# angelocatalani/neural-network-compression

Measured on AMD Instinct MI355X. Metric: weights/sec through prune+k-means (K=256), higher is better.
Workload: dtype f32

## Files before the change

neural_network_compression_amd/csrc/nnc_hip.hip:

```cpp
#include "nnc_common.hpp"
#include "nnc_km_shared.hpp"


extern "C" size_t nnc_kmeans_workspace_bytes(int32_t k)
{
    (void)k;
    return sizeof(KmWs) + 256;
}

extern "C" int32_t nnc_fix_shift(float absmax, int64_t n_total)
{
    int L = 1;
    while (((int64_t)1 << L) < n_total && L < 62) L++;
    if (!(absmax > 0.0f) || !std::isfinite(absmax)) return 0;
    int P = 0;
    (void)std::frexp((double)absmax, &P);
    return std::min(28, 62 - L) - P;
}

__device__ __forceinline__ int fix_f32(float v, int Sft)
{
    return (int)rintf(ldexpf(v, Sft));
}

// ... 911 lines not shown
        tab = &ws->tab[ws->cur];
        src.zr = ws->bnd.zr; src.zl = ws->bnd.zl; src.cand = ws->bnd.cand; src.orig = ws->bnd.orig; src.ku = &ws->bnd.ku;
    }
    KmBndPre<BR> pre;
    const bool fixed_src = !(which & 1);
    if (fixed_src) km_bounds_preload<BR>(pre, j, lane, ws, src);
    const int stop = (which & 2) ? 0 : (ws->st.done | ws->st.paused);
    const int unasked = (which & 4) ? !ws->wide : 0;
    const int hint = ws->help_hint;
    const float mean = ws->p.x_mean;
    const int Sft = ws->p.fix_shift;
    if (stop | unasked) return;
    int qn_seen = 0;
    if (!fixed_src) km_bounds_preload<BR>(pre, j, lane, ws, src);
    const bool published = km_bounds_wave<BR>(j, lane, xs, n, ws, tab, src, mean, Sft, pblk, &qn_seen, pre, hint == 2, &wg_searched);
    KBSTAMP(16 * j + 5, 0);
    const bool waits = hint == 2 && !published && fixed_src;
    int looks = 0;
    if (waits) {
        const int nwaves = pre.ku;
        for (int nap = 0; nap < 64 && __builtin_amdgcn_s_memrealtime() - t_enter < 900ull; nap++) __builtin_amdgcn_s_sleep(16);
        for (int look = 0; look < 128; look++) {
            looks++;
            if (km_peek_i(&ws->q_searched) >= nwaves) break;
            __builtin_amdgcn_s_sleep(48);
        }
    }
    KBSTAMP(16 * j + 7, 0);
    if (NNC_KM_TRACE_PTR && lane == 0) NNC_KM_TRACE_PTR[16 * j + 12] = (unsigned long long)looks;
    if (published || hint || uni_i(qn_seen) > 0) km_bounds_help(lane, xs, ws, tab, mean, Sft, j, hint == 2 ? pre.ku : 0);
    KBSTAMP(16 * j + 6, 0);
}

__global__ __launch_bounds__(256) void k_prefix_blocks(const float *__restrict__ xs, long long n, float mean, int Sft, long long *__restrict__ pblk)
{
    const int lane = threadIdx.x & 63;
    const long long nblk = (n + KM_PB - 1) / KM_PB;
    long long *__restrict__ pfine = pblk + km_pfine_off(n);
    const long long wave = (long long)blockIdx.x * 4 + (threadIdx.x >> 6), nwaves = (long long)gridDim.x * 4;
    for (long long b0 = wave; b0 < nblk; b0 += 4 * nwaves) {
        float4 v[4];
        bool full[4], have[4];
#pragma unroll
        for (int u = 0; u < 4; u++) {
            const long long b = b0 + u * nwaves;
            have[u] = b < nblk;
            full[u] = have[u] && (b + 1) * KM_PB <= n;
            v[u] = full[u] ? *reinterpret_cast<const float4 *>(xs + b * KM_PB + 4 * lane) : make_float4(0.f, 0.f, 0.f, 0.f);
        }
#pragma unroll
        for (int u = 0; u < 4; u++) {
            if (!have[u]) continue;
            const long long b = b0 + u * nwaves;
            const long long i0 = b * KM_PB + 4 * lane;
            long long acc = 0;
            if (full[u]) {
                acc = ((long long)fix_f32(v[u].x - mean, Sft) + fix_f32(v[u].y - mean, Sft)) + ((long long)fix_f32(v[u].z - mean, Sft) + fix_f32(v[u].w - mean, Sft));
            } else {
                for (int q = 0; q < 4; q++) if (i0 + q < n) acc += fix_f32(xs[i0 + q] - mean, Sft);
            }
#pragma unroll
            for (int off = 1; off <= 8; off <<= 1) acc += __shfl_xor(acc, off);
            if ((lane & 15) == 0) pfine[4 * b + (lane >> 4)] = acc;
            acc += __shfl_xor(acc, 16);
            acc += __shfl_xor(acc, 32);
            if (lane == 0) pblk[b] = acc;
        }
    }
    if (blockIdx.x == 0 && threadIdx.x == 0) pblk[nblk] = 0;
}

__global__ __launch_bounds__(256) void k_prefix_fine(long long *__restrict__ pblk, long long n)
{
    const long long nblk = km_prefix_nblk(n);
    const long long *__restrict__ pgrp = km_pgrp(pblk, n);
    long long *__restrict__ pfine = pblk + km_pfine_off(n);
    const long long b = (long long)blockIdx.x * 256 + threadIdx.x;
    if (b > nblk) return;
    const long long base = pblk[b] + pgrp[b / KM_PG];
    if (b == nblk) { pfine[4 * b] = base; return; }
    const long long q0 = pfine[4 * b], q1 = pfine[4 * b + 1], q2 = pfine[4 * b + 2];
    pfine[4 * b] = base; pfine[4 * b + 1] = base + q0; pfine[4 * b + 2] = base + q0 + q1; pfine[4 * b + 3] = base + q0 + q1 + q2;
}

__global__ __launch_bounds__(KM_THREADS) void k_prefix_groups(long long *__restrict__ pblk, long long nblk, long long *__restrict__ pgrp)
{
    __shared__ long long wave_tot[KM_THREADS / 64];
// ... 998 lines not shown
    HIPCHK(hipMemcpy(out8, reinterpret_cast<KmWs *>(ws)->kl_trace, 24 * sizeof(unsigned long long), hipMemcpyDeviceToHost));
    return NNC_OK;
}

extern "C" int nnc_debug_set_trace(unsigned long long *buf_dev)
{
    HIPCHK(hipMemcpyToSymbol(HIP_SYMBOL(g_km_trace), &buf_dev, sizeof(buf_dev)));
    unsigned long long *fin = buf_dev ? buf_dev + 6 * 1024 : nullptr;
    HIPCHK(hipMemcpyToSymbol(HIP_SYMBOL(g_fin_trace), &fin, sizeof(fin)));
    return NNC_OK;
}

extern "C" int nnc_debug_clock(int blocks, int iters, float *out_dev, void *stream)
{
    hipLaunchKernelGGL(k_debug_clock, dim3(blocks), dim3(256), 0, S(stream), iters, out_dev);
    LAUNCHCHK("k_debug_clock");
    return NNC_OK;
}

static int g_ablation = 0;
static int g_deal = []() { const char *e = getenv("NNC_KM_DEAL"); return e ? atoi(e) : 1; }();
extern "C" int nnc_debug_set_ablation(int a) { g_ablation = a; return NNC_OK; }
#else
static const int g_ablation = 0, g_deal = 1;
#endif

extern "C" size_t nnc_kmeans_prefix_bytes(int64_t n)
{
    if (n < 0) return 0;
    const long long nblk = (n + KM_PB - 1) / KM_PB;
    return (size_t)(nblk + 2 + (nblk + 1 + KM_PG - 1) / KM_PG + 2 + 4 * (nblk + 1) + 4) * sizeof(long long);
}

extern "C" int nnc_kmeans_prefix_build(const float *x_sorted, const nnc_kmeans_params *p, int64_t *prefix_dev, void *stream)
{
    if (!p || !prefix_dev || p->n < 0 || (p->n > 0 && !x_sorted)) return fail(NNC_EINVAL, "nnc_kmeans_prefix_build: bad argument");
    if ((reinterpret_cast<uintptr_t>(x_sorted) & 15) != 0 || (reinterpret_cast<uintptr_t>(prefix_dev) & 7) != 0)
        return fail(NNC_EINVAL, "nnc_kmeans_prefix_build: x_sorted must be 16-byte aligned, prefix_dev 8-byte aligned");
    if (p->n >= ((int64_t)1 << 40)) return fail(NNC_EINVAL, "nnc_kmeans_prefix_build: n >= 2^40");
    const long long nblk = (p->n + KM_PB - 1) / KM_PB;
    long long *pb = reinterpret_cast<long long *>(prefix_dev);
    const int grid = (int)std::max<long long>(1, std::min<long long>((nblk + 3) / 4, (long long)cu_count() * 8));
    NNC_LAUNCH_PROF(NNC_PROF_PREFIX, k_prefix_blocks, dim3(grid), dim3(256), 0, S(stream), x_sorted, (long long)p->n, p->x_mean, p->fix_shift, pb);
    LAUNCHCHK("k_prefix_blocks");
    const long long ngroups = (nblk + 1 + KM_PG - 1) / KM_PG;
    long long *pg = pb + nblk + 2;
    if (ngroups > 0) {
        hipLaunchKernelGGL(k_prefix_groups, dim3((unsigned)ngroups), dim3(KM_THREADS), 0, S(stream), pb, nblk, pg);
        LAUNCHCHK("k_prefix_groups");
    }
    hipLaunchKernelGGL(k_prefix_top, dim3(1), dim3(KM_THREADS), 0, S(stream), pg, ngroups);
    LAUNCHCHK("k_prefix_top");
    hipLaunchKernelGGL(k_prefix_fine, dim3((unsigned)((nblk + 1 + 255) / 256)), dim3(256), 0, S(stream), pb, (long long)p->n);
    LAUNCHCHK("k_prefix_fine");
    return NNC_OK;
}

int km_launch_accumulate(const float *x, KmWs *w, const nnc_kmeans_params *p, void *stream, int which)
{
    if (p->prefix_dev && p->n > 0) {
        if ((reinterpret_cast<uintptr_t>(x) & 15) != 0) return fail(NNC_EINVAL, "rank-boundary iteration: the sorted vector must be 16-byte aligned");
        const int nb = (p->k + 3) / 4;
        const long long *pb = reinterpret_cast<const long long *>(p->prefix_dev);
#define KM_LAUNCH_BOUNDS(BR) NNC_LAUNCH_PROF(NNC_PROF_BOUNDS, (k_bounds<BR>), dim3(nb), dim3(256), 0, S(stream), x, (long long)p->n, w, which, pb)
        if (p->k <= 64) KM_LAUNCH_BOUNDS(1);
        else if (p->k <= 128) KM_LAUNCH_BOUNDS(2);
        else if (p->k <= 256) KM_LAUNCH_BOUNDS(4);
        else if (p->k <= 512) KM_LAUNCH_BOUNDS(8);
        else if (p->k <= 1024) KM_LAUNCH_BOUNDS(16);
        else KM_LAUNCH_BOUNDS(KM_BND_R);
#undef KM_LAUNCH_BOUNDS
        LAUNCHCHK("k_bounds");
        return NNC_OK;
    }
    int glog2, rlog2;
    km_defaults(p, &glog2, &rlog2);
// ... 1386 lines not shown
```

neural_network_compression_amd/csrc/nnc_layer.hip:

```cpp
#include <hip/hip_runtime.h>

#include <algorithm>
#include <cmath>
#include <cstdint>
#include <cstring>
#include <string>
#include <vector>

#include "nnc.h"

int nnc_set_error_(int code, const char *msg);
int nnc_publish_bytes_(const void *src_dev, void *dst_host_mapped, int nbytes, void *host_ticket, uint64_t ticket, void *stream);
int nnc_wait_ticket_(void *host_ticket, uint64_t ticket, void *stream);
int nnc_sort_pruned_bounded_flagged_(const float *x, int64_t n, int64_t n_neg, int64_t n_zero, float vmin, float vmax, float thr,
                                     float *sorted_out, void *ws, size_t ws_bytes, int32_t *flag_dev, void *stream);

extern "C" int nnc_host_linspace_f32(float start, float stop, int32_t num, float *out)
{
    if (num < 0 || (num > 0 && !out)) return nnc_set_error_(NNC_EINVAL, "nnc_host_linspace_f32: bad argument");
    if (num == 0) return NNC_OK;
    const int div = num - 1;
    const volatile float delta = stop - start;
    if (div > 0) {
        const volatile float step = delta / (float)div;
        for (int i = 0; i < num; i++) {
            volatile float y = (float)i;
            if (step == 0.0f) { y = y / (float)div; y = y * delta; }
            else y = y * step;
            y = y + start;
            out[i] = y;
        }
        out[num - 1] = stop;
    } else {
        volatile float y = 0.0f;
        y = y * delta;
        y = y + start;
        out[0] = y;
    }
    return NNC_OK;
}

static void linspace_f64(double start, double stop, int num, double *out)
{
    const int div = num - 1;
    const volatile double delta = stop - start;
    if (div > 0) {
        const volatile double step = delta / (double)div;
        for (int i = 0; i < num; i++) {
// ... 243 lines not shown
            if (!std::isfinite(min_nz)) {
                LHIP(hipStreamWaitEvent(s, side->join, 0));
                LHIP(hipStreamSynchronize(s));
                side_join.joined = true;
                if (lp->prune) { res->sigma = h_prune[0]; res->threshold = h_prune[1]; res->n_zeroed = h_nz[0]; }
                res->status = NNC_LAYER_HOST;
                return NNC_OK;
            }
            LCHK(nnc_host_linspace_f32(min_nz, max_nz, 32, steps));
            std::memcpy(h_steps, steps, 128);
            LCHK(nnc_rank_sorted_f32(xs, n, h_steps, 32, ranks_d, stream));
        }
        const uint64_t t_rk = ++(*ticket_io);
        LCHK(nnc_publish_bytes_(out6 + 2, hb + 512 + 8, 56 + 33 * 8 + 16, h_ticket, t_rk, stream));
        LCHK(nnc_wait_ticket_(h_ticket_side, t_mv, side->stream));
        LHIP(hipStreamWaitEvent(s, side->join, 0));
        side_join.joined = true;
        const float mean = h_mv[0], var = h_mv[1];
        if (!std::isfinite(mean) || !std::isfinite(var) || !std::isfinite(xmin) || !std::isfinite(xmax)) {
            LCHK(nnc_wait_ticket_(h_ticket, t_rk, stream));
            if (lp->prune) { res->sigma = h_prune[0]; res->threshold = h_prune[1]; res->n_zeroed = h_nz[0]; }
            res->status = NNC_LAYER_HOST;
            return NNC_OK;
        }
        nnc_kmeans_params p;
        std::memset(&p, 0, sizeof(p));
        const volatile float tol = var * 1e-4f;
        const volatile float lo = xmin - mean, hi = xmax - mean;
        p.n = n; p.n_total = n; p.k = k; p.max_iter = 300;
        p.fix_shift = nnc_fix_shift(std::max(std::fabs((float)lo), std::fabs((float)hi)), n);
        p.grid_log2 = 0; p.replicas_log2 = -1; p.flags = lp->km_flags & (NNC_KM_TWO_LAUNCH | NNC_KM_LOOP);
        p.x_mean = mean; p.tol = tol; p.lo = lo; p.hi = hi;
        if (with_prefix) {
            LCHK(nnc_kmeans_prefix_build(xs, &p, reinterpret_cast<int64_t *>(wb + L.prefix), stream));
            p.prefix_dev = reinterpret_cast<int64_t *>(wb + L.prefix);
        }
        LCHK(nnc_wait_ticket_(h_ticket, t_rk, stream));
        if (bounded && *h_oob) {
            if (lp->prune) { res->sigma = h_prune[0]; res->threshold = h_prune[1]; res->n_zeroed = h_nz[0]; }
            res->status = NNC_LAYER_HOST;
            return NNC_OK;
        }
        if (lp->mode == NNC_INIT_LINEAR) {
            LCHK(nnc_host_linspace_f32(xmin, xmax, k, space));
        } else {
            int64_t counts31[31];
            for (int b = 0; b < 31; b++) counts31[b] = h_ranks[b + 1] - h_ranks[b];
            for (int b = 0; b < 31; b++)
                if (steps[b] <= 0.0f && 0.0f < steps[b + 1]) { counts31[b] -= n_zero; break; }
            float xnew[300];
            double cdf[300];
            LCHK(nnc_host_cdf(steps, counts31, xnew, cdf));
            LCHK(nnc_host_density_init(xnew, cdf, lp->bits, space));
        }
        std::memcpy(h_space, space, (size_t)k * 4);
        LCHK(nnc_kmeans_init(wb + L.km_ws, L.km_ws_bytes, &p, h_space, stream));
        nnc_kmeans_status st;
        std::memset(&st, 0, sizeof(st));
        int32_t nwin = 0;
        LCHK(nnc_kmeans_fit(xs, wb + L.km_ws, &p, 16, 1, L.reloc_bytes ? wb + L.reloc : nullptr, L.reloc_bytes, hb, ticket_io, &st, &nwin, stream));
        if (!st.done) {
            if (lp->prune) { res->sigma = h_prune[0]; res->threshold = h_prune[1]; res->n_zeroed = h_nz[0]; }
            res->status = NNC_LAYER_HOST;
            return NNC_OK;
        }
        LCHK(nnc_kmeans_get_centers(wb + L.km_ws, 0, 0, centers_d, stream));
        LCHK(nnc_kmeans_assign(x, wb + L.km_ws, &p, 0, labels_out, res->label_bytes, lp->want_values ? values_out : nullptr, nullptr, nullptr, stream));
// ... 15 lines not shown
```

neural_network_compression_amd/csrc/nnc_sort.hip:

```cpp
#include <hip/hip_runtime.h>
#include <cmath>
#include <cstdlib>
#include <cstring>

#include <algorithm>
#include <string>

#include "nnc.h"

extern "C" const char *nnc_last_error(void);
int nnc_set_error_(int code, const char *msg);

#ifndef OS_THREADS
#define OS_THREADS 1024
#endif
#define OS_WAVES (OS_THREADS / 64)
#ifndef OS_ITEMS
#define OS_ITEMS 16
#endif
#ifndef OS_BLOCKS_PER_CU
#define OS_BLOCKS_PER_CU 1
#endif
#ifndef OS_RANK_LDS
#define OS_RANK_LDS 1
#endif
#define OS_TILE (OS_THREADS * OS_ITEMS)
#define OS_MAXBITS 9
#define OS_MAXR (1 << OS_MAXBITS)
#define OS_MAXPASS 4
#define OS_SPIN_LIMIT (1 << 22)
#define OSP_THREADS 1024
#define OSP_PER 16
#define OSP_TILE (OSP_THREADS * OSP_PER)

__device__ __forceinline__ unsigned f32_ord(float v)
{
    const unsigned b = __float_as_uint(v);
    return (b & 0x80000000u) ? ~b : (b | 0x80000000u);
}
__device__ __forceinline__ float f32_unord(unsigned o)
{
    return __uint_as_float((o & 0x80000000u) ? (o ^ 0x80000000u) : ~o);
}

struct OsMap { unsigned lo_neg, hi_neg, lo_pos, hi_pos, span_neg; int bounded; };
struct OsPlan { int passes; int shift[OS_MAXPASS]; int rb[OS_MAXPASS]; };

__device__ __forceinline__ unsigned os_key(const OsMap &m, float e, bool &outside)
{
    const unsigned o = f32_ord(e);
    if (!m.bounded) return o;
    if (e < 0.0f) { outside |= (o < m.lo_neg) | (o > m.hi_neg); const unsigned c = o < m.lo_neg ? m.lo_neg : (o > m.hi_neg ? m.hi_neg : o); return c - m.lo_neg; }
    outside |= (o < m.lo_pos) | (o > m.hi_pos);
    const unsigned c = o < m.lo_pos ? m.lo_pos : (o > m.hi_pos ? m.hi_pos : o);
    return m.span_neg + (c - m.lo_pos);
}
__device__ __forceinline__ float os_value(const OsMap &m, unsigned k)
{
    if (!m.bounded) return f32_unord(k);
    return f32_unord(k < m.span_neg ? k + m.lo_neg : k - m.span_neg + m.lo_pos);
}

#define OS_CTRL_WORDS 4

template <bool SKIPZ>
__global__ __launch_bounds__(OSP_THREADS) void k_os_prep(const float *__restrict__ x, long long n, unsigned *__restrict__ keys,
                                                         unsigned long long *__restrict__ ctrl, long long cap, OsMap km, int rb0, unsigned *__restrict__ ghist)
{
    __shared__ unsigned comp_s[SKIPZ ? OSP_TILE : 1];
    __shared__ unsigned hist_s[OS_MAXR];
    __shared__ unsigned wave_tot[OSP_THREADS / 64];
    __shared__ unsigned long long base_s;
    const int tid = threadIdx.x, lane = tid & 63, wv = tid >> 6;
    for (int i = tid; i < OS_MAXR; i += OSP_THREADS) hist_s[i] = 0u;
    __syncthreads();
    const bool vec = (reinterpret_cast<uintptr_t>(x) & 15) == 0;
    const float4 *x4 = reinterpret_cast<const float4 *>(x);
    const unsigned mask0 = (1u << rb0) - 1u;
    bool outside = false;
    const long long ntiles = (n + OSP_TILE - 1) / OSP_TILE;
    auto load_tile = [&](long long tt, float (&e)[OSP_PER]) {
        const long long tile0 = tt * OSP_TILE;
        if (tt >= ntiles) return;
        if (vec && tile0 + OSP_TILE <= n) {
#pragma unroll
            for (int j = 0; j < OSP_PER / 4; j++) {
                const float4 q = x4[(tile0 >> 2) + (long long)j * OSP_THREADS + tid];
                e[4 * j] = q.x; e[4 * j + 1] = q.y; e[4 * j + 2] = q.z; e[4 * j + 3] = q.w;
            }
        } else {
#pragma unroll
            for (int j = 0; j < OSP_PER; j++) {
                const long long i = tile0 + (long long)j * OSP_THREADS + tid;
                e[j] = i < n ? x[i] : 0.0f;
            }
        }
    };
    float en[OSP_PER];
    load_tile(blockIdx.x, en);
    for (long long t = blockIdx.x; t < ntiles; t += gridDim.x) {
        const long long tile0 = t * OSP_TILE;
        const bool fast = vec && tile0 + OSP_TILE <= n;
        float e[OSP_PER];
#pragma unroll
        for (int j = 0; j < OSP_PER; j++) e[j] = en[j];
        load_tile(t + gridDim.x, en);
        unsigned key[OSP_PER];
        unsigned take = 0;
#pragma unroll
        for (int j = 0; j < OSP_PER; j++) {
            bool ok = SKIPZ ? !(e[j] == 0.0f) : true;
            if (!SKIPZ && !fast) ok = tile0 + (long long)j * OSP_THREADS + tid < n;
            key[j] = 0u;
            if (ok) { key[j] = os_key(km, e[j], outside); take |= 1u << j; }
        }
#pragma unroll
        for (int j = 0; j < OSP_PER; j++)
            if (take & (1u << j)) atomicAdd(&hist_s[key[j] & mask0], 1u);
        if (SKIPZ) {
            const unsigned c = (unsigned)__popc(take);
            unsigned sc = c;
            for (int off = 1; off < 64; off <<= 1) { const unsigned o = __shfl_up(sc, off); if (lane >= off) sc += o; }
            if (lane == 63) wave_tot[wv] = sc;
            __syncthreads();
            unsigned pre = 0, tot = 0;
            for (int w = 0; w < OSP_THREADS / 64; w++) { const unsigned o = wave_tot[w]; if (w < wv) pre += o; tot += o; }
            if (tid == 0) base_s = atomicAdd(ctrl, (unsigned long long)tot);
            unsigned at = pre + sc - c;
#pragma unroll
            for (int j = 0; j < OSP_PER; j++)
                if (take & (1u << j)) comp_s[at++] = key[j];
            __syncthreads();
            const long long base = (long long)base_s;
            for (unsigned i = tid; i < tot; i += OSP_THREADS)
                if (base + i < cap) keys[base + i] = comp_s[i];
            __syncthreads();
        }
    }
    if (outside) atomicOr(ctrl + 1, 1ull);
    __syncthreads();
    for (int i = tid; i < OS_MAXR; i += OSP_THREADS) {
        const unsigned v = hist_s[i];
        if (v) atomicAdd(&ghist[i], v);
    }
}

#ifdef NNC_DIAG
__device__ unsigned long long *g_os_trace = nullptr;
extern "C" int nnc_debug_os_trace(void *buf)
{
    unsigned long long *p = reinterpret_cast<unsigned long long *>(buf);
    return hipMemcpyToSymbol(HIP_SYMBOL(g_os_trace), &p, sizeof(p)) == hipSuccess ? NNC_OK : NNC_EHIP;
}
#define OS_STAMP(i) do { if (g_os_trace && t == 0) g_os_trace[((size_t)pass * 8192 + (size_t)(tile < 8192 ? tile : 8191)) * 8 + (i)] = __builtin_amdgcn_s_memrealtime(); } while (0)
#else
#define OS_STAMP(i) do { } while (0)
#endif

__device__ __forceinline__ void os_publish(unsigned long long *w, unsigned tag, unsigned v)
{
    __hip_atomic_store(w, ((unsigned long long)tag << 32) | v, __ATOMIC_RELAXED, __HIP_MEMORY_SCOPE_AGENT);
}
__device__ __forceinline__ unsigned long long os_peek(const unsigned long long *w)
{
    return __hip_atomic_load(w, __ATOMIC_RELAXED, __HIP_MEMORY_SCOPE_AGENT);
}

template <int RB, bool FULL>
__device__ __forceinline__ void os_peers(unsigned d, bool valid, unsigned &plo, unsigned &phi)
{
    const unsigned long long all = FULL ? ~0ull : __ballot(valid);
    plo = (unsigned)all; phi = (unsigned)(all >> 32);
#pragma unroll
    for (int b = 0; b < RB; b++) {
        const int m = ((int)(d << (31 - b))) >> 31;
        const unsigned long long mb = FULL ? __ballot(m != 0) : __ballot(valid && m != 0);
        plo &= ~((unsigned)mb ^ (unsigned)m);
        phi &= ~((unsigned)(mb >> 32) ^ (unsigned)m);
    }
}

#ifndef OS_LOOK
#define OS_LOOK 4
#endif

template <int RB, int SRC, int DST>
__global__ __launch_bounds__(OS_THREADS, OS_BLOCKS_PER_CU * OS_THREADS / 256) void k_os_pass(const void *__restrict__ in_, void *__restrict__ out_, long long n, int shift, int pass, int nrb,
                                                           const unsigned *__restrict__ ghist, unsigned *__restrict__ ghist_next, unsigned long long *__restrict__ status,
                                                           unsigned long long *__restrict__ ctrl, OsMap km, long long n_neg, long long n_zero, int abl)
{
    constexpr int R = 1 << RB;
    constexpr unsigned MASK = (unsigned)R - 1u;
    constexpr int DPT = (R + OS_THREADS - 1) / OS_THREADS;
    __shared__ unsigned keys_s[OS_TILE];
    __shared__ unsigned short wcnt[OS_WAVES][R];
    __shared__ unsigned short tpre[R];
    __shared__ unsigned gpos[R];
    __shared__ unsigned gdig[R];
    __shared__ unsigned nhist[OS_MAXR];
    __shared__ unsigned wsum[OS_WAVES];
    __shared__ long long tile_s;
    const int t = threadIdx.x, lane = t & 63, wv = t >> 6;
    const unsigned *in_k = reinterpret_cast<const unsigned *>(in_);
    const float *in_f = reinterpret_cast<const float *>(in_);
    unsigned *out_k = reinterpret_cast<unsigned *>(out_);
    float *out_f = reinterpret_cast<float *>(out_);
    const unsigned tagA = 2u * (unsigned)pass + 1u, tagP = tagA + 1u;
    unsigned *ticket = reinterpret_cast<unsigned *>(ctrl + 2) + pass;
    const int nshift = shift + RB;
    const unsigned nmask = nrb > 0 ? (1u << nrb) - 1u : 0u;
    {
        unsigned v[DPT], own = 0;
#pragma unroll
        for (int r = 0; r < DPT; r++) { const int d = t * DPT + r; v[r] = d < R ? ghist[d] : 0u; own += v[r]; }
        unsigned sc = own;
        for (int off = 1; off < 64; off <<= 1) { const unsigned o = __shfl_up(sc, off); if (lane >= off) sc += o; }
        if (lane == 63) wsum[wv] = sc;
        for (int i = t; i < OS_MAXR; i += OS_THREADS) nhist[i] = 0u;
        __syncthreads();
        unsigned run = sc - own;
        for (int w = 0; w < wv; w++) run += wsum[w];
#pragma unroll
        for (int r = 0; r < DPT; r++) { const int d = t * DPT + r; if (d < R) gdig[d] = run; run += v[r]; }
// ... 144 lines not shown
                            __builtin_amdgcn_s_sleep(1);
                        } else polls = 0;
                    }
                }
                os_publish(&status[(size_t)tile * R + d], tagP, excl + tc[r]);
            }
            gpos[d] = gdig[d] + excl - (unsigned)tpre[d];
        }
        OS_STAMP(4);
        __syncthreads();
        OS_STAMP(5);
        for (int j = t; j < cnt_tile; j += OS_THREADS) {
            const unsigned kv = keys_s[j];
            const unsigned d = (kv >> shift) & MASK;
            const unsigned r = gpos[d] + (unsigned)j;
            if ((long long)r < n && !(abl & 4)) {
                if (DST == 0) out_k[r] = kv;
                else out_f[(long long)r + ((long long)r >= n_neg ? n_zero : 0)] = os_value(km, kv);
            }
        }
        OS_STAMP(6);
        __syncthreads();
        OS_STAMP(7);
    }
    if (gave_up) atomicOr(ctrl + 1, 2ull);
    if (nrb > 0) {
        for (int i = t; i <= (int)nmask; i += OS_THREADS) {
            const unsigned v = nhist[i];
            if (v) atomicAdd(&ghist_next[i], v);
        }
    }
}

static unsigned host_ord(float v)
{
    unsigned b;
    std::memcpy(&b, &v, 4);
    return (b & 0x80000000u) ? ~b : (b | 0x80000000u);
}

static size_t al256(size_t b) { return (b + 255) & ~(size_t)255; }

static int os_cus()
{
    static int cus[64] = {0};
    int dev = 0;
    if (hipGetDevice(&dev) != hipSuccess || dev < 0 || dev >= 64) return 256;
    if (!cus[dev]) {
        int v = 0;
        if (hipDeviceGetAttribute(&v, hipDeviceAttributeMultiprocessorCount, dev) != hipSuccess || v <= 0) v = 256;
        cus[dev] = v;
    }
    return cus[dev];
}

static OsPlan os_plan(int bits)
{
    OsPlan pl;
    std::memset(&pl, 0, sizeof(pl));
    int rb;
    if (bits <= 8) { pl.passes = 1; rb = 8; }
    else if (bits <= 16) { pl.passes = 2; rb = 8; }
    else if (bits <= 18) { pl.passes = 2; rb = 9; }
    else if (bits <= 24) { pl.passes = 3; rb = 8; }
    else if (bits <= 27) { pl.passes = 3; rb = 9; }
    else { pl.passes = 4; rb = 8; }
    for (int p = 0; p < pl.passes; p++) { pl.shift[p] = p * rb; pl.rb[p] = rb; }
    return pl;
}

static size_t os_status_bytes(int64_t n_keys)
{
    const int64_t ntiles = (n_keys + OS_TILE - 1) / OS_TILE;
    return al256((size_t)std::max<int64_t>(ntiles, 1) * OS_MAXR * 8);
}
static size_t os_ws_bytes(int64_t n_keys)
{
    return 2 * al256((size_t)n_keys * 4 + 16) + al256(OS_CTRL_WORDS * 8) + al256((size_t)(OS_MAXPASS + 1) * OS_MAXR * 4) + os_status_bytes(n_keys) + 256;
}
static unsigned char *os_ws_base(void *ws) { return reinterpret_cast<unsigned char *>((reinterpret_cast<uintptr_t>(ws) + 255) & ~(uintptr_t)255); }

static int os_sort(const float *x, int64_t n, bool skip_zeros, int64_t n_neg, int64_t n_zero, const OsMap &km, int bits, float *sorted_out, void *ws,
                   size_t ws_bytes, int32_t *flag_dev, const char *who, void *stream)
{
    const int64_t n_keys = skip_zeros ? n - n_zero : n;
    if (!ws || ws_bytes < os_ws_bytes(n_keys)) return nnc_set_error_(NNC_ENOSPACE, (std::string(who) + ": workspace too small").c_str());
    hipStream_t s = reinterpret_cast<hipStream_t>(stream);
    unsigned char *b = os_ws_base(ws);
    unsigned *ka = reinterpret_cast<unsigned *>(b); b += al256((size_t)n_keys * 4 + 16);
    unsigned *kb = reinterpret_cast<unsigned *>(b); b += al256((size_t)n_keys * 4 + 16);
    unsigned long long *ctrl = reinterpret_cast<unsigned long long *>(b); b += al256(OS_CTRL_WORDS * 8);
    unsigned *ghist = reinterpret_cast<unsigned *>(b); b += al256((size_t)(OS_MAXPASS + 1) * OS_MAXR * 4);
    unsigned long long *status = reinterpret_cast<unsigned long long *>(b);
    hipError_t e;
    const size_t zero_bytes = al256(OS_CTRL_WORDS * 8) + al256((size_t)(OS_MAXPASS + 1) * OS_MAXR * 4) + os_status_bytes(n_keys);
    if ((e = hipMemsetAsync(ctrl, 0, zero_bytes, s)) != hipSuccess) return nnc_set_error_(NNC_EHIP, hipGetErrorString(e));
    if (skip_zeros && n_zero > 0 && n_keys == 0 && (e = hipMemsetAsync(sorted_out + n_neg, 0, (size_t)n_zero * 4, s)) != hipSuccess) return nnc_set_error_(NNC_EHIP, hipGetErrorString(e));
    const OsPlan pl = os_plan(bits);
    int abl = 0;
#ifdef NNC_DIAG
    { const char *ev = getenv("NNC_OS_ABLATE"); abl = ev ? atoi(ev) : 0; }
#endif
    if (n_keys > 0) {
        const long long ptiles = (n + OSP_TILE - 1) / OSP_TILE;
        const int pgrid = (int)std::min<long long>(std::max<long long>(ptiles, 1), 2LL * os_cus());
        if (skip_zeros) hipLaunchKernelGGL((k_os_prep<true>), dim3(pgrid), dim3(OSP_THREADS), 0, s, x, (long long)n, ka, ctrl, (long long)n_keys, km, pl.rb[0], ghist);
        else hipLaunchKernelGGL((k_os_prep<false>), dim3(pgrid), dim3(OSP_THREADS), 0, s, x, (long long)n, (unsigned *)nullptr, ctrl, (long long)n_keys, km, pl.rb[0], ghist);
        if ((e = hipGetLastError()) != hipSuccess) return nnc_set_error_(NNC_EHIP, hipGetErrorString(e));
        const long long ntiles = (n_keys + OS_TILE - 1) / OS_TILE;
        const int grid = (int)std::min<long long>(ntiles, (long long)OS_BLOCKS_PER_CU * os_cus());
        const void *src = skip_zeros ? (const void *)ka : (const void *)x;
        unsigned *dst = skip_zeros ? kb : ka;
        for (int p = 0; p < pl.passes; p++) {
            const bool first_f = (p == 0 && !skip_zeros), last = (p == pl.passes - 1);
            void *o = last ? (void *)sorted_out : (void *)dst;
#define OS_LAUNCH(SRC, DST) do { \
                if (pl.rb[p] == 9) hipLaunchKernelGGL((k_os_pass<9, SRC, DST>), dim3(grid), dim3(OS_THREADS), 0, s, src, o, (long long)n_keys, pl.shift[p], p, last ? 0 : pl.rb[p + 1], \
                                                      ghist + (size_t)p * OS_MAXR, ghist + (size_t)(p + 1) * OS_MAXR, status, ctrl, km, (long long)(skip_zeros ? n_neg : n_keys), (long long)(skip_zeros ? n_zero : 0), abl); \
                else hipLaunchKernelGGL((k_os_pass<8, SRC, DST>), dim3(grid), dim3(OS_THREADS), 0, s, src, o, (long long)n_keys, pl.shift[p], p, last ? 0 : pl.rb[p + 1], \
                                        ghist + (size_t)p * OS_MAXR, ghist + (size_t)(p + 1) * OS_MAXR, status, ctrl, km, (long long)(skip_zeros ? n_neg : n_keys), (long long)(skip_zeros ? n_zero : 0), abl); \
            } while (0)
            if (first_f && last) OS_LAUNCH(1, 1);
            else if (first_f) OS_LAUNCH(1, 0);
            else if (last) OS_LAUNCH(0, 1);
            else OS_LAUNCH(0, 0);
#undef OS_LAUNCH
            if ((e = hipGetLastError()) != hipSuccess) return nnc_set_error_(NNC_EHIP, hipGetErrorString(e));
            src = dst;
            dst = (dst == ka) ? kb : ka;
        }
    }
    if (flag_dev && (e = hipMemcpyAsync(flag_dev, reinterpret_cast<unsigned char *>(ctrl) + 8, 4, hipMemcpyDeviceToDevice, s)) != hipSuccess)
        return nnc_set_error_(NNC_EHIP, hipGetErrorString(e));
    return NNC_OK;
}

static OsMap os_identity()
{
    OsMap m;
    std::memset(&m, 0, sizeof(m));
    return m;
}

extern "C" size_t nnc_sort_workspace_bytes(int64_t n) { return n <= 0 ? 0 : os_ws_bytes(n); }

extern "C" int nnc_sort_f32(const float *x, int64_t n, float *sorted_out, void *ws, size_t ws_bytes, void *stream)
{
    if (n < 0 || n >= ((int64_t)1 << 31) || (n > 0 && (!x || !sorted_out))) return nnc_set_error_(NNC_EINVAL, "nnc_sort_f32: bad argument");
    if (n == 0) return NNC_OK;
    return os_sort(x, n, false, 0, 0, os_identity(), 32, sorted_out, ws, ws_bytes, nullptr, "nnc_sort_f32", stream);
}

extern "C" size_t nnc_sort_pruned_workspace_bytes(int64_t n, int64_t n_neg, int64_t n_zero)
// ... 81 lines not shown
```

Measured before the change: 10.03 billion.

## Add MSD two-pass sort path and skip loading known-zero prefix blocks

Adds an MSD radix sort for large bounded pruned inputs. A top-bucket scatter kernel writes the zero fill during its pass, and a per-bucket shared-memory finish kernel places the keys. If any bucket is too skewed, it sets a flag and falls back to the existing LSD passes, which now early-exit unless that flag is set. Separately, the prefix-block kernel no longer reads blocks known to hold pruned zeros and writes their constant fixed-point sums directly. The LSD passes are still launched as guards, and the new sort path adds complexity around the skew fallback.

```diff
diff --git a/neural_network_compression_amd/csrc/nnc_hip.hip b/neural_network_compression_amd/csrc/nnc_hip.hip
--- a/neural_network_compression_amd/csrc/nnc_hip.hip
+++ b/neural_network_compression_amd/csrc/nnc_hip.hip
@@ -967,27 +967,35 @@
     KBSTAMP(16 * j + 6, 0);
 }
 
-__global__ __launch_bounds__(256) void k_prefix_blocks(const float *__restrict__ xs, long long n, float mean, int Sft, long long *__restrict__ pblk)
+__global__ __launch_bounds__(256) void k_prefix_blocks(const float *__restrict__ xs, long long n, float mean, int Sft, long long *__restrict__ pblk, long long z0, long long z1)
 {
     const int lane = threadIdx.x & 63;
     const long long nblk = (n + KM_PB - 1) / KM_PB;
+    const long long zb0 = (z0 + KM_PB - 1) / KM_PB, zb1 = z1 / KM_PB;
+    const long long zfix = fix_f32(0.0f - mean, Sft);
     long long *__restrict__ pfine = pblk + km_pfine_off(n);
     const long long wave = (long long)blockIdx.x * 4 + (threadIdx.x >> 6), nwaves = (long long)gridDim.x * 4;
     for (long long b0 = wave; b0 < nblk; b0 += 4 * nwaves) {
         float4 v[4];
-        bool full[4], have[4];
+        bool full[4], have[4], zeros[4];
 #pragma unroll
         for (int u = 0; u < 4; u++) {
             const long long b = b0 + u * nwaves;
             have[u] = b < nblk;
             full[u] = have[u] && (b + 1) * KM_PB <= n;
-            v[u] = full[u] ? *reinterpret_cast<const float4 *>(xs + b * KM_PB + 4 * lane) : make_float4(0.f, 0.f, 0.f, 0.f);
+            zeros[u] = full[u] && b >= zb0 && b < zb1;
+            v[u] = (full[u] && !zeros[u]) ? *reinterpret_cast<const float4 *>(xs + b * KM_PB + 4 * lane) : make_float4(0.f, 0.f, 0.f, 0.f);
         }
 #pragma unroll
         for (int u = 0; u < 4; u++) {
             if (!have[u]) continue;
             const long long b = b0 + u * nwaves;
             const long long i0 = b * KM_PB + 4 * lane;
+            if (zeros[u]) {
+                if ((lane & 15) == 0) pfine[4 * b + (lane >> 4)] = 64 * zfix;
+                if (lane == 0) pblk[b] = KM_PB * zfix;
+                continue;
+            }
             long long acc = 0;
             if (full[u]) {
                 acc = ((long long)fix_f32(v[u].x - mean, Sft) + fix_f32(v[u].y - mean, Sft)) + ((long long)fix_f32(v[u].z - mean, Sft) + fix_f32(v[u].w - mean, Sft));
@@ -2052,7 +2060,13 @@
     return (size_t)(nblk + 2 + (nblk + 1 + KM_PG - 1) / KM_PG + 2 + 4 * (nblk + 1) + 4) * sizeof(long long);
 }
 
+int nnc_kmeans_prefix_build_zeros_(const float *x_sorted, const nnc_kmeans_params *p, int64_t *prefix_dev, int64_t z0, int64_t z1, void *stream);
 extern "C" int nnc_kmeans_prefix_build(const float *x_sorted, const nnc_kmeans_params *p, int64_t *prefix_dev, void *stream)
+{
+    return nnc_kmeans_prefix_build_zeros_(x_sorted, p, prefix_dev, 0, 0, stream);
+}
+
+int nnc_kmeans_prefix_build_zeros_(const float *x_sorted, const nnc_kmeans_params *p, int64_t *prefix_dev, int64_t z0, int64_t z1, void *stream)
 {
     if (!p || !prefix_dev || p->n < 0 || (p->n > 0 && !x_sorted)) return fail(NNC_EINVAL, "nnc_kmeans_prefix_build: bad argument");
     if ((reinterpret_cast<uintptr_t>(x_sorted) & 15) != 0 || (reinterpret_cast<uintptr_t>(prefix_dev) & 7) != 0)
@@ -2061,7 +2075,8 @@
     const long long nblk = (p->n + KM_PB - 1) / KM_PB;
     long long *pb = reinterpret_cast<long long *>(prefix_dev);
     const int grid = (int)std::max<long long>(1, std::min<long long>((nblk + 3) / 4, (long long)cu_count() * 8));
-    NNC_LAUNCH_PROF(NNC_PROF_PREFIX, k_prefix_blocks, dim3(grid), dim3(256), 0, S(stream), x_sorted, (long long)p->n, p->x_mean, p->fix_shift, pb);
+    NNC_LAUNCH_PROF(NNC_PROF_PREFIX, k_prefix_blocks, dim3(grid), dim3(256), 0, S(stream), x_sorted, (long long)p->n, p->x_mean, p->fix_shift, pb,
+                    (long long)(z0 >= 0 && z0 <= z1 && z1 <= p->n ? z0 : 0), (long long)(z0 >= 0 && z0 <= z1 && z1 <= p->n ? z1 : 0));
     LAUNCHCHK("k_prefix_blocks");
     const long long ngroups = (nblk + 1 + KM_PG - 1) / KM_PG;
     long long *pg = pb + nblk + 2;
diff --git a/neural_network_compression_amd/csrc/nnc_layer.hip b/neural_network_compression_amd/csrc/nnc_layer.hip
--- a/neural_network_compression_amd/csrc/nnc_layer.hip
+++ b/neural_network_compression_amd/csrc/nnc_layer.hip
@@ -14,6 +14,7 @@
 int nnc_wait_ticket_(void *host_ticket, uint64_t ticket, void *stream);
 int nnc_sort_pruned_bounded_flagged_(const float *x, int64_t n, int64_t n_neg, int64_t n_zero, float vmin, float vmax, float thr,
                                      float *sorted_out, void *ws, size_t ws_bytes, int32_t *flag_dev, void *stream);
+int nnc_kmeans_prefix_build_zeros_(const float *x_sorted, const nnc_kmeans_params *p, int64_t *prefix_dev, int64_t z0, int64_t z1, void *stream);
 
 extern "C" int nnc_host_linspace_f32(float start, float stop, int32_t num, float *out)
 {
@@ -323,7 +324,7 @@
         p.grid_log2 = 0; p.replicas_log2 = -1; p.flags = lp->km_flags & (NNC_KM_TWO_LAUNCH | NNC_KM_LOOP);
         p.x_mean = mean; p.tol = tol; p.lo = lo; p.hi = hi;
         if (with_prefix) {
-            LCHK(nnc_kmeans_prefix_build(xs, &p, reinterpret_cast<int64_t *>(wb + L.prefix), stream));
+            LCHK(nnc_kmeans_prefix_build_zeros_(xs, &p, reinterpret_cast<int64_t *>(wb + L.prefix), n_neg, n_neg + n_zero, stream));
             p.prefix_dev = reinterpret_cast<int64_t *>(wb + L.prefix);
         }
         LCHK(nnc_wait_ticket_(h_ticket, t_rk, stream));
diff --git a/neural_network_compression_amd/csrc/nnc_sort.hip b/neural_network_compression_amd/csrc/nnc_sort.hip
--- a/neural_network_compression_amd/csrc/nnc_sort.hip
+++ b/neural_network_compression_amd/csrc/nnc_sort.hip
@@ -32,6 +32,21 @@
 #define OSP_THREADS 1024
 #define OSP_PER 16
 #define OSP_TILE (OSP_THREADS * OSP_PER)
+#define MS_MAXT 13
+#define MS_MAXNB (1 << MS_MAXT)
+#define MS_MINT 10
+#define MS_MAXLOW 14
+#define MS_MINBITS 16
+#ifndef MS_MIN_KEYS
+#define MS_MIN_KEYS (1 << 19)
+#endif
+#ifndef MS_SKEW_LIMIT
+#define MS_SKEW_LIMIT 49152u
+#endif
+#define MSF_THREADS 512
+#define MSF_WAVES (MSF_THREADS / 64)
+#define MSF_STAGE 8192
+#define OS_FLAG_LSD (1ull << 32)
 
 __device__ __forceinline__ unsigned f32_ord(float v)
 {
@@ -65,18 +80,19 @@
 
 template <bool SKIPZ>
 __global__ __launch_bounds__(OSP_THREADS) void k_os_prep(const float *__restrict__ x, long long n, unsigned *__restrict__ keys,
-                                                         unsigned long long *__restrict__ ctrl, long long cap, OsMap km, int rb0, unsigned *__restrict__ ghist)
+                                                         unsigned long long *__restrict__ ctrl, long long cap, OsMap km, int hshift, int hbits, unsigned *__restrict__ ghist)
 {
     __shared__ unsigned comp_s[SKIPZ ? OSP_TILE : 1];
-    __shared__ unsigned hist_s[OS_MAXR];
+    __shared__ unsigned hist_s[SKIPZ ? MS_MAXNB : OS_MAXR];
     __shared__ unsigned wave_tot[OSP_THREADS / 64];
     __shared__ unsigned long long base_s;
     const int tid = threadIdx.x, lane = tid & 63, wv = tid >> 6;
-    for (int i = tid; i < OS_MAXR; i += OSP_THREADS) hist_s[i] = 0u;
+    const int hbins = 1 << hbits;
+    for (int i = tid; i < hbins; i += OSP_THREADS) hist_s[i] = 0u;
     __syncthreads();
     const bool vec = (reinterpret_cast<uintptr_t>(x) & 15) == 0;
     const float4 *x4 = reinterpret_cast<const float4 *>(x);
-    const unsigned mask0 = (1u << rb0) - 1u;
+    const unsigned mask0 = (unsigned)hbins - 1u;
     bool outside = false;
     const long long ntiles = (n + OSP_TILE - 1) / OSP_TILE;
     auto load_tile = [&](long long tt, float (&e)[OSP_PER]) {
@@ -116,7 +132,7 @@
         }
 #pragma unroll
         for (int j = 0; j < OSP_PER; j++)
-            if (take & (1u << j)) atomicAdd(&hist_s[key[j] & mask0], 1u);
+            if (take & (1u << j)) atomicAdd(&hist_s[(key[j] >> hshift) & mask0], 1u);
         if (SKIPZ) {
             const unsigned c = (unsigned)__popc(take);
             unsigned sc = c;
@@ -139,7 +155,7 @@
     }
     if (outside) atomicOr(ctrl + 1, 1ull);
     __syncthreads();
-    for (int i = tid; i < OS_MAXR; i += OSP_THREADS) {
+    for (int i = tid; i < hbins; i += OSP_THREADS) {
         const unsigned v = hist_s[i];
         if (v) atomicAdd(&ghist[i], v);
     }
@@ -187,8 +203,9 @@
 template <int RB, int SRC, int DST>
 __global__ __launch_bounds__(OS_THREADS, OS_BLOCKS_PER_CU * OS_THREADS / 256) void k_os_pass(const void *__restrict__ in_, void *__restrict__ out_, long long n, int shift, int pass, int nrb,
                                                            const unsigned *__restrict__ ghist, unsigned *__restrict__ ghist_next, unsigned long long *__restrict__ status,
-                                                           unsigned long long *__restrict__ ctrl, OsMap km, long long n_neg, long long n_zero, int abl)
-{
+                                                           unsigned long long *__restrict__ ctrl, OsMap km, long long n_neg, long long n_zero, int abl, int guard)
+{
+    if (guard && !(ctrl[1] & OS_FLAG_LSD)) return;
     constexpr int R = 1 << RB;
     constexpr unsigned MASK = (unsigned)R - 1u;
     constexpr int DPT = (R + OS_THREADS - 1) / OS_THREADS;
@@ -399,6 +416,221 @@
     }
 }
 
+__global__ __launch_bounds__(OS_THREADS) void k_ms_scatter(const unsigned *__restrict__ keys, unsigned *__restrict__ out, long long n, int lowb, int tb,
+                                                           unsigned *__restrict__ region, unsigned long long *__restrict__ ctrl, int rb0, unsigned *__restrict__ ghist0,
+                                                           float *__restrict__ zero_out, long long n_zero)
+{
+    __shared__ unsigned keys_s[OS_TILE];
+    __shared__ unsigned base_s[MS_MAXNB];
+    __shared__ unsigned cnt_s[MS_MAXNB];
+    __shared__ unsigned short tpre_s[MS_MAXNB];
+    __shared__ unsigned wsum[OS_WAVES], wmax[OS_WAVES];
+    constexpr int MAXDPT = MS_MAXNB / OS_THREADS;
+    const int t = threadIdx.x, lane = t & 63, wv = t >> 6;
+    const int nb = 1 << tb, dpt = nb / OS_THREADS;
+    const unsigned *__restrict__ tophist = region;
+    unsigned *__restrict__ cursor = region + nb;
+    unsigned *__restrict__ bases = region + 2 * (size_t)nb;
+    unsigned v[MAXDPT], own = 0, big = 0;
+#pragma unroll
+    for (int r = 0; r < MAXDPT; r++) { v[r] = r < dpt ? tophist[t * dpt + r] : 0u; own += v[r]; big = v[r] > big ? v[r] : big; }
+    unsigned sc = own;
+    for (int off = 1; off < 64; off <<= 1) { const unsigned o = __shfl_up(sc, off); if (lane >= off) sc += o; }
+    for (int off = 32; off > 0; off >>= 1) { const unsigned o = __shfl_xor(big, off); big = o > big ? o : big; }
+    if (lane == 63) wsum[wv] = sc;
+    if (lane == 0) wmax[wv] = big;
+    __syncthreads();
+    unsigned run = sc - own;
+    for (int w = 0; w < OS_WAVES; w++) { if (w < wv) run += wsum[w]; big = wmax[w] > big ? wmax[w] : big; }
+    const long long ntiles = (n + OS_TILE - 1) / OS_TILE;
+    if (big > MS_SKEW_LIMIT) {
+        if (blockIdx.x == 0 && t == 0) atomicOr(ctrl + 1, OS_FLAG_LSD);
+        const int r0 = 1 << rb0;
+        for (int i = t; i < r0; i += OS_THREADS) cnt_s[i] = 0u;
+        __syncthreads();
+        for (long long tile = blockIdx.x; tile < ntiles; tile += gridDim.x) {
+            const long long tile0 = tile * OS_TILE;
+#pragma unroll
+            for (int i = 0; i < OS_ITEMS; i++) {
+                const long long idx = tile0 + i * OS_THREADS + t;
+                if (idx < n) atomicAdd(&cnt_s[keys[idx] & (unsigned)(r0 - 1)], 1u);
+            }
+        }
+        __syncthreads();
+        for (int i = t; i < r0; i += OS_THREADS) { const unsigned c = cnt_s[i]; if (c) atomicAdd(&ghist0[i], c); }
+        return;
+    }
+#pragma unroll
+    for (int r = 0; r < MAXDPT; r++)
+        if (r < dpt) { base_s[t * dpt + r] = run; if (blockIdx.x == 0) bases[t * dpt + r] = run; run += v[r]; }
+    if (blockIdx.x == 0 && t == OS_THREADS - 1) bases[nb] = run;
+    for (long long tile = blockIdx.x; tile < ntiles; tile += gridDim.x) {
+        const long long tile0 = tile * OS_TILE;
+        const int cnt_tile = (int)((n - tile0) < OS_TILE ? (n - tile0) : OS_TILE);
+        for (int d = t; d < nb; d += OS_THREADS) cnt_s[d] = 0u;
+        unsigned key[OS_ITEMS];
+#pragma unroll
+        for (int i = 0; i < OS_ITEMS; i++) {
+            const int idx = i * OS_THREADS + t;
+            key[i] = idx < cnt_tile ? keys[tile0 + idx] : 0u;
+        }
+        __syncthreads();
+        unsigned short rnk[OS_ITEMS];
+#pragma unroll
+        for (int i = 0; i < OS_ITEMS; i++) {
+            const unsigned d = min(key[i] >> lowb, (unsigned)nb - 1u);
+            rnk[i] = 0;
+            if (i * OS_THREADS + t < cnt_tile) rnk[i] = (unsigned short)atomicAdd(&cnt_s[d], 1u);
+        }
+        __syncthreads();
+        {
+            unsigned c[MAXDPT], mine = 0;
+#pragma unroll
+            for (int r = 0; r < MAXDPT; r++) { c[r] = r < dpt ? cnt_s[t * dpt + r] : 0u; mine += c[r]; }
+            unsigned s2 = mine;
+            for (int off = 1; off < 64; off <<= 1) { const unsigned o = __shfl_up(s2, off); if (lane >= off) s2 += o; }
+            if (lane == 63) wsum[wv] = s2;
+            __syncthreads();
+            unsigned at = s2 - mine;
+            for (int w = 0; w < wv; w++) at += wsum[w];
+#pragma unroll
+            for (int r = 0; r < MAXDPT; r++)
+                if (r < dpt) { tpre_s[t * dpt + r] = (unsigned short)at; at += c[r]; }
+        }
+        __syncthreads();
+#pragma unroll
+        for (int i = 0; i < OS_ITEMS; i++) {
+            const unsigned d = min(key[i] >> lowb, (unsigned)nb - 1u);
+            if (i * OS_THREADS + t < cnt_tile) keys_s[(unsigned)tpre_s[d] + (unsigned)rnk[i]] = key[i];
+        }
+        {
+            unsigned c[MAXDPT], got[MAXDPT];
+#pragma unroll
+            for (int r = 0; r < MAXDPT; r++) {
+                const int d = (t + r * OS_THREADS + (int)blockIdx.x * 64) & (nb - 1);
+                c[r] = r < dpt ? cnt_s[d] : 0u;
+            }
+#pragma unroll
+            for (int r = 0; r < MAXDPT; r++) {
+                const int d = (t + r * OS_THREADS + (int)blockIdx.x * 64) & (nb - 1);
+                got[r] = c[r] ? atomicAdd(&cursor[d], c[r]) : 0u;
+            }
+#pragma unroll
+            for (int r = 0; r < MAXDPT; r++) {
+                const int d = (t + r * OS_THREADS + (int)blockIdx.x * 64) & (nb - 1);
+                if (c[r]) cnt_s[d] = base_s[d] + got[r] - (unsigned)tpre_s[d];
+            }
+        }
+        if (n_zero > 0) {
+            const long long per = ((n_zero + ntiles - 1) / ntiles + 3) & ~3ll;
+            const long long z0 = tile * per, z1 = (z0 + per < n_zero) ? z0 + per : n_zero;
+            if ((reinterpret_cast<uintptr_t>(zero_out) & 15) == 0) {
+                for (long long i = z0 + 4ll * t; i + 3 < z1; i += 4ll * OS_THREADS) *reinterpret_cast<float4 *>(zero_out + i) = make_float4(0.f, 0.f, 0.f, 0.f);
+                if (t == 0) for (long long i = z0 + ((z1 - z0 > 0 ? z1 - z0 : 0) & ~3ll); i < z1; i++) zero_out[i] = 0.0f;
+            } else {
+                for (long long i = z0 + t; i < z1; i += OS_THREADS) zero_out[i] = 0.0f;
+            }
+        }
+        __syncthreads();
+#pragma unroll 4
+        for (int j = t; j < cnt_tile; j += OS_THREADS) {
+            const unsigned kv = keys_s[j];
+            const unsigned d = min(kv >> lowb, (unsigned)nb - 1u);
+            const unsigned pos = cnt_s[d] + (unsigned)j;
+            if ((long long)pos < n) out[pos] = kv;
+        }
+    }
+}
+
+#define MSF_UNPACK(q) {(q).x & 0xFFFFu, (q).x >> 16, (q).y & 0xFFFFu, (q).y >> 16, (q).z & 0xFFFFu, (q).z >> 16, (q).w & 0xFFFFu, (q).w >> 16}
+
+__global__ __launch_bounds__(MSF_THREADS, 2 * MSF_THREADS / 256) void k_ms_finish(const unsigned *__restrict__ keys, float *__restrict__ out, long long n, int lowb, int tb,
+                                                                                   unsigned *__restrict__ region, const unsigned long long *__restrict__ ctrl, OsMap km,
+                                                                                   long long n_neg, long long n_zero)
+{
+    static_assert(MS_SKEW_LIMIT <= 65535u, "the finish counts and places a bucket's keys in 16 bits");
+    constexpr int KR = 8;
+    __shared__ __align__(16) unsigned hist_s[(1 << MS_MAXLOW) / 2];
+    __shared__ float stage_s[MSF_STAGE];
+    __shared__ unsigned wtot[MSF_WAVES];
+    const int t = threadIdx.x, lane = t & 63, wv = t >> 6;
+    const int nb = 1 << tb;
+    if (ctrl[1] & OS_FLAG_LSD) {
+        const long long words = 3ll * nb + 1;
+        for (long long i = (long long)blockIdx.x * MSF_THREADS + t; i < words; i += (long long)gridDim.x * MSF_THREADS) region[i] = 0u;
+        return;
+    }
+    const unsigned *__restrict__ bases = region + 2 * (size_t)nb;
+    const unsigned lowmask = (1u << lowb) - 1u;
+    const int G = (1 << lowb) / 8;
+    int gwl = lowb - 3 - 3;
+    if (gwl < 6) gwl = 6;
+    const int GW = 1 << gwl;
+    for (int b = blockIdx.x; b < nb; b += gridDim.x) {
+        const long long lo = bases[b];
+        long long hi = bases[b + 1];
+        if (hi > n) hi = n;
+        if (hi <= lo) continue;
+        const long long cnt = hi - lo;
+        for (int g = t; g < G; g += MSF_THREADS) reinterpret_cast<uint4 *>(hist_s)[g] = make_uint4(0u, 0u, 0u, 0u);
+        unsigned k[KR];
+#pragma unroll
+        for (int u = 0; u < KR; u++) { const long long i = lo + u * MSF_THREADS + t; k[u] = i < hi ? keys[i] : 0u; }
+        __syncthreads();
+#pragma unroll
+        for (int u = 0; u < KR; u++)
+            if (lo + u * MSF_THREADS + t < hi) { const unsigned d = k[u] & lowmask; atomicAdd(&hist_s[d >> 1], 1u << ((d & 1u) * 16u)); }
+        for (long long i = lo + KR * MSF_THREADS + t; i < hi; i += MSF_THREADS) { const unsigned d = keys[i] & lowmask; atomicAdd(&hist_s[d >> 1], 1u << ((d & 1u) * 16u)); }
+        __syncthreads();
+        {
+            unsigned carry = 0;
+            for (int g0 = wv * GW; g0 < (wv + 1) * GW && g0 < G; g0 += 64) {
+                const int g = g0 + lane;
+                uint4 q = make_uint4(0u, 0u, 0u, 0u);
+                if (g < G) q = reinterpret_cast<const uint4 *>(hist_s)[g];
+                const unsigned c[8] = MSF_UNPACK(q);
+                const unsigned s = ((c[0] + c[1]) + (c[2] + c[3])) + ((c[4] + c[5]) + (c[6] + c[7]));
+                unsigned sc = s;
+                for (int off = 1; off < 64; off <<= 1) { const unsigned o = __shfl_up(sc, off); if (lane >= off) sc += o; }
+                const unsigned p0 = carry + sc - s;
+                carry += __shfl(sc, 63);
+                const unsigned p1 = p0 + c[0], p2 = p1 + c[1], p3 = p2 + c[2], p4 = p3 + c[3], p5 = p4 + c[4], p6 = p5 + c[5], p7 = p6 + c[6];
+                if (g < G) reinterpret_cast<uint4 *>(hist_s)[g] = make_uint4(p0 | (p1 << 16), p2 | (p3 << 16), p4 | (p5 << 16), p6 | (p7 << 16));
+            }
+            if (lane == 0) wtot[wv] = carry;
+        }
+        __syncthreads();
+        unsigned wt[MSF_WAVES];
+#pragma unroll
+        for (int w = 0; w < MSF_WAVES; w++) wt[w] = wtot[w];
+        const bool staged = cnt <= MSF_STAGE;
+        auto place = [&](unsigned key) {
+            const unsigned d = key & lowmask, sh = (d & 1u) * 16u;
+            const int seg = (int)(d >> 3) >> gwl;
+            unsigned pos = (atomicAdd(&hist_s[d >> 1], 1u << sh) >> sh) & 0xFFFFu;
+#pragma unroll
+            for (int w = 0; w < MSF_WAVES - 1; w++) pos += w < seg ? wt[w] : 0u;
+            const float val = os_value(km, key);
+            if (staged) { if (pos < (unsigned)MSF_STAGE) stage_s[pos] = val; }
+            else {
+                const long long r = lo + pos;
+                if (r < hi) out[r + (r >= n_neg ? n_zero : 0)] = val;
+            }
+        };
+#pragma unroll
+        for (int u = 0; u < KR; u++)
+            if (lo + u * MSF_THREADS + t < hi) place(k[u]);
+        for (long long i = lo + KR * MSF_THREADS + t; i < hi; i += MSF_THREADS) place(keys[i]);
+        __syncthreads();
+        if (staged)
+            for (long long a = t; a < cnt; a += MSF_THREADS) {
+                const long long r = lo + a;
+                out[r + (r >= n_neg ? n_zero : 0)] = stage_s[a];
+            }
+        __syncthreads();
+    }
+}
+
 static unsigned host_ord(float v)
 {
     unsigned b;
@@ -444,6 +676,11 @@
 static size_t os_ws_bytes(int64_t n_keys)
 {
     return 2 * al256((size_t)n_keys * 4 + 16) + al256(OS_CTRL_WORDS * 8) + al256((size_t)(OS_MAXPASS + 1) * OS_MAXR * 4) + os_status_bytes(n_keys) + 256;
+}
+static int64_t os_ms_min_keys()
+{
+    static const int64_t v = [] { const char *ev = getenv("NNC_MS_MIN_KEYS"); return ev && *ev ? (int64_t)atoll(ev) : (int64_t)MS_MIN_KEYS; }();
+    return v;
 }
 static unsigned char *os_ws_base(void *ws) { return reinterpret_cast<unsigned char *>((reinterpret_cast<uintptr_t>(ws) + 255) & ~(uintptr_t)255); }
 
@@ -464,6 +701,9 @@
     if ((e = hipMemsetAsync(ctrl, 0, zero_bytes, s)) != hipSuccess) return nnc_set_error_(NNC_EHIP, hipGetErrorString(e));
     if (skip_zeros && n_zero > 0 && n_keys == 0 && (e = hipMemsetAsync(sorted_out + n_neg, 0, (size_t)n_zero * 4, s)) != hipSuccess) return nnc_set_error_(NNC_EHIP, hipGetErrorString(e));
     const OsPlan pl = os_plan(bits);
+    const int ms_tb = std::max(bits - MS_MAXLOW, MS_MINT), ms_lowb = bits - ms_tb;
+    const bool msd = skip_zeros && km.bounded && bits >= MS_MINBITS && ms_tb <= MS_MAXT && n_keys >= os_ms_min_keys() &&
+                     os_status_bytes(n_keys) >= (3 * ((size_t)1 << ms_tb) + 1) * 4;
     int abl = 0;
 #ifdef NNC_DIAG
     { const char *ev = getenv("NNC_OS_ABLATE"); abl = ev ? atoi(ev) : 0; }
@@ -471,11 +711,20 @@
     if (n_keys > 0) {
         const long long ptiles = (n + OSP_TILE - 1) / OSP_TILE;
         const int pgrid = (int)std::min<long long>(std::max<long long>(ptiles, 1), 2LL * os_cus());
-        if (skip_zeros) hipLaunchKernelGGL((k_os_prep<true>), dim3(pgrid), dim3(OSP_THREADS), 0, s, x, (long long)n, ka, ctrl, (long long)n_keys, km, pl.rb[0], ghist);
-        else hipLaunchKernelGGL((k_os_prep<false>), dim3(pgrid), dim3(OSP_THREADS), 0, s, x, (long long)n, (unsigned *)nullptr, ctrl, (long long)n_keys, km, pl.rb[0], ghist);
+        unsigned *region = reinterpret_cast<unsigned *>(status);
+        if (msd) hipLaunchKernelGGL((k_os_prep<true>), dim3(pgrid), dim3(OSP_THREADS), 0, s, x, (long long)n, ka, ctrl, (long long)n_keys, km, ms_lowb, ms_tb, region);
+        else if (skip_zeros) hipLaunchKernelGGL((k_os_prep<true>), dim3(pgrid), dim3(OSP_THREADS), 0, s, x, (long long)n, ka, ctrl, (long long)n_keys, km, 0, pl.rb[0], ghist);
+        else hipLaunchKernelGGL((k_os_prep<false>), dim3(pgrid), dim3(OSP_THREADS), 0, s, x, (long long)n, (unsigned *)nullptr, ctrl, (long long)n_keys, km, 0, pl.rb[0], ghist);
         if ((e = hipGetLastError()) != hipSuccess) return nnc_set_error_(NNC_EHIP, hipGetErrorString(e));
         const long long ntiles = (n_keys + OS_TILE - 1) / OS_TILE;
         const int grid = (int)std::min<long long>(ntiles, (long long)OS_BLOCKS_PER_CU * os_cus());
+        if (msd) {
+            hipLaunchKernelGGL(k_ms_scatter, dim3(grid), dim3(OS_THREADS), 0, s, ka, kb, (long long)n_keys, ms_lowb, ms_tb, region, ctrl, pl.rb[0], ghist, sorted_out + n_neg, (long long)n_zero);
+            if ((e = hipGetLastError()) != hipSuccess) return nnc_set_error_(NNC_EHIP, hipGetErrorString(e));
+            const int fgrid = std::min(1 << ms_tb, 2 * os_cus());
+            hipLaunchKernelGGL(k_ms_finish, dim3(fgrid), dim3(MSF_THREADS), 0, s, kb, sorted_out, (long long)n_keys, ms_lowb, ms_tb, region, ctrl, km, (long long)n_neg, (long long)n_zero);
+            if ((e = hipGetLastError()) != hipSuccess) return nnc_set_error_(NNC_EHIP, hipGetErrorString(e));
+        }
         const void *src = skip_zeros ? (const void *)ka : (const void *)x;
         unsigned *dst = skip_zeros ? kb : ka;
         for (int p = 0; p < pl.passes; p++) {
@@ -483,9 +732,9 @@
             void *o = last ? (void *)sorted_out : (void *)dst;
 #define OS_LAUNCH(SRC, DST) do { \
                 if (pl.rb[p] == 9) hipLaunchKernelGGL((k_os_pass<9, SRC, DST>), dim3(grid), dim3(OS_THREADS), 0, s, src, o, (long long)n_keys, pl.shift[p], p, last ? 0 : pl.rb[p + 1], \
-                                                      ghist + (size_t)p * OS_MAXR, ghist + (size_t)(p + 1) * OS_MAXR, status, ctrl, km, (long long)(skip_zeros ? n_neg : n_keys), (long long)(skip_zeros ? n_zero : 0), abl); \
+                                                      ghist + (size_t)p * OS_MAXR, ghist + (size_t)(p + 1) * OS_MAXR, status, ctrl, km, (long long)(skip_zeros ? n_neg : n_keys), (long long)(skip_zeros ? n_zero : 0), abl, msd ? 1 : 0); \
                 else hipLaunchKernelGGL((k_os_pass<8, SRC, DST>), dim3(grid), dim3(OS_THREADS), 0, s, src, o, (long long)n_keys, pl.shift[p], p, last ? 0 : pl.rb[p + 1], \
-                                        ghist + (size_t)p * OS_MAXR, ghist + (size_t)(p + 1) * OS_MAXR, status, ctrl, km, (long long)(skip_zeros ? n_neg : n_keys), (long long)(skip_zeros ? n_zero : 0), abl); \
+                                        ghist + (size_t)p * OS_MAXR, ghist + (size_t)(p + 1) * OS_MAXR, status, ctrl, km, (long long)(skip_zeros ? n_neg : n_keys), (long long)(skip_zeros ? n_zero : 0), abl, msd ? 1 : 0); \
             } while (0)
             if (first_f && last) OS_LAUNCH(1, 1);
             else if (first_f) OS_LAUNCH(1, 0);
```

Measured after the change: 7.377 billion. -26.5%, worse.
